# IRVLab/so_dso_place_recognition

Hardware: AMD Instinct MI355X
Metric: queries/sec over 100k-signature DB (SC 20x60, z-score fusion, top-1) (higher is better)
Workload: dtype f16x2 (fp32 carried as f16 hi + lo, fp32 accumulate); binary intensity channel: one f16 product per term, rounded to its exact integer count; 1 GPU; sc_match_100k; db_signatures=100000, descriptor=SC 20x60 x 2 channels, mask_width=0, k=1, db_rows_per_gpu=100000

## Files before the change

so_dso_place_recognition_amd/csrc/kernels.hpp:

```cpp
#pragma once
#include <hip/hip_runtime.h>
#include <stdint.h>

struct pr_ctx;

namespace pr {

constexpr int SC_NF = 31;
constexpr int SC_NSLOT = 16;
constexpr int SC_QIMG = SC_NF * 320;
constexpr int SC_DSTEP = 640;
constexpr int SC_DIMG = 2 * SC_NSLOT * SC_DSTEP;
__host__ __device__ inline int sc_fpos(int f) { return f == 0 ? 0 : (f == 30 ? 1 : f + 1); }
constexpr int SCH_QBLK = 1288;
constexpr int SCH_QIMG = SC_NF * SCH_QBLK;
constexpr int SCH_DTILE = 768;
constexpr int SCH_DFREQ = 4 * SCH_DTILE;
constexpr int SCH_DIMG = SC_NF * SCH_DFREQ;
__host__ __device__ constexpr int sch_qlo_byte(int ring) { return 40 + ((ring + 4) % 20) * 2; }
__host__ __device__ constexpr int sch_a1_byte(int k) { return k == 3 ? 0 : 16 * k; }
__host__ __device__ constexpr int sch_a2_byte(int k) { return k == 0 ? 48 : k == 1 ? 64 : k == 2 ? 32 : 16; }
__host__ __device__ constexpr int sch_b1_byte(int lane) { return lane < 48 ? lane * 16 : SCH_DTILE + (lane - 48) * 16; }
__host__ __device__ constexpr int sch_b2_byte(int lane) { return lane < 32 ? lane * 16 : lane < 48 ? SCH_DTILE + lane * 16 : SCH_DTILE + (lane - 32) * 16; }
constexpr int SCF_QBLK = 640;
constexpr int SCF_QIMG = SC_NF * SCF_QBLK;
constexpr int SCF_DFREQ = 2 * SCH_DTILE;
constexpr int SCF_DIMG = SC_NF * SCF_DFREQ;
constexpr int M2_TILE = 96 * 64;

inline int sc_qgroups8(int m) { return ((m + 31) / 32) * 4; }
inline int sc_qgroups8_f16(int m) { return ((m + 63) / 64) * 8; }
inline int sc_dgroups(int n) { return (n + 15) / 16; }
inline int m2_tiles(int sigs) { return (sigs + 7) / 8; }
inline int m2_qtiles(int sigs) { return ((m2_tiles(sigs) + 11) / 12) * 12; }

constexpr int SC_BSTAT_INTS = 8;
struct ScBin {
  const int* qstat; const int* dstat;
  const float* qinfo; const float* dinfo;
  int* viol;
  int gen;
  float bconst;
  float pair_scale;
  int gate;
  int chsel;
};
#ifdef __HIPCC__
__device__ __forceinline__ bool sc_bin_bound(const ScBin& b, float& bound) {
  const int q0 = b.qstat[0], q1 = b.qstat[1], d0 = b.dstat[0], d1 = b.dstat[1];
  const float eq = __builtin_sqrtf(((__int_as_float(b.qstat[2]) + __int_as_float(b.qstat[3])) + __int_as_float(b.qstat[4])) + __int_as_float(b.qstat[5]));
  const float ed = __builtin_sqrtf(((__int_as_float(b.dstat[2]) + __int_as_float(b.dstat[3])) + __int_as_float(b.dstat[4])) + __int_as_float(b.dstat[5]));
  bound = (eq + ed + eq * ed + b.bconst * (1.f + eq) * (1.f + ed)) * 1.001f;
  return q0 == 0 && d0 == 0 && bound * __builtin_sqrtf((float)q1 * (float)d1) < 0.72f;
}
#endif
void launch_sc_pack(hipStream_t st, const void* sig, int dtype, int rows, int role, float* packed, int groups,
                    const double* twiddle, int* flags, int* bad);
void launch_sc_match(hipStream_t st, const float* qpk, int m, const float* dpk, int n, const float* cst,
                     float* d_p, float* d_i, int nsplit_override);
size_t sc_match_lds_bytes();
void launch_zero_ints(hipStream_t st, int* p, int n);
void launch_fill_ints(hipStream_t st, int* p, int n, int v);
void launch_sc_pack_h(hipStream_t st, const void* sig, int dtype, int rows, int role, void* packed, int groups,
                      const double* twiddle, int* flags, int* bad, int single = 0,
                      float* binfo = nullptr, int* bstat = nullptr);
void launch_sc_pack_h_rows(hipStream_t st, const void* sig, int dtype, int rows, int row0, void* packed, int groups, const double* twiddle,
                           int* flags, int* bad, int single, float* binfo, int* bstat);
void launch_sc_match_h(hipStream_t st, const void* qpk, int m, const void* dpk, int n, const void* cst, float* d_p,
// ... 262 lines not shown
```

so_dso_place_recognition_amd/csrc/sc_match_e.hip:

```cpp
#include <cstdlib>
#include <cstring>

#include "kernels.hpp"
#ifndef E_NO_WAIT1
#define E_WAIT1
#endif
#ifndef E_NO_ACC_OPERANDS
#define E_BACC
#define E_AACC
#define E_SPLIT3
#ifndef E_BD
#define E_BD 5
#endif
#ifndef E_AD
#define E_AD 3
#endif
#ifndef E_PARKR
#define E_PARKR 1
#endif
#endif
#ifndef E_BD
#define E_BD 4
#endif
#ifndef E_BD1
#define E_BD1 8
#endif

namespace pr {
namespace {

typedef _Float16 f16x2 __attribute__((ext_vector_type(2)));
typedef float f32x2 __attribute__((ext_vector_type(2)));
typedef float f32x4 __attribute__((ext_vector_type(4)));
typedef float f32x16 __attribute__((ext_vector_type(16)));
typedef unsigned u32x2 __attribute__((ext_vector_type(2)));
typedef unsigned u32x4 __attribute__((ext_vector_type(4)));
typedef u32x4 u32x4_a8 __attribute__((aligned(8)));

struct AOps { u32x4 h, l; };
struct BOps { u32x4 reh, rel, imh, iml; };
enum { A_H = 0, A_L = 1 };
enum { B_REH = 0, B_REL = 1, B_IMH = 2, B_IML = 3 };

__host__ __device__ constexpr int seqf(int P) { return 16 * (P >> 4) + ((P & 15) >> 1) + 8 * (P & 1); }

typedef const u32x4_a8 __attribute__((address_space(3))) * lds_tile_p;
template <int T>
__device__ __forceinline__ void load_a(AOps& a, unsigned addr) {
  const u32x4 v = *reinterpret_cast<lds_tile_p>(addr);
  if (T == A_H) a.h = v; else a.l = v;
}
template <bool LO, int F, int T, bool SV = false>
__device__ __forceinline__ void load_b(BOps& b, __amdgpu_buffer_rsrc_t rs, int voff) {
  constexpr int soff = LO ? F * SCH_DFREQ : SV ? F * SCH_DFREQ + (T == B_IMH ? 2 : 0) * SCH_DTILE : F * SCF_DFREQ + (T == B_IMH ? 1 : 0) * SCH_DTILE,
                ioff = LO ? ((T == B_IMH || T == B_IML) ? 2 * SCH_DTILE : 0) : 0;
#ifdef E_ABL_ONE_B
  if (!LO && T == B_IMH) { b.imh = b.reh; return; }
#endif
#ifdef E_ABL_B_HOT
  const u32x4 v = __builtin_amdgcn_raw_buffer_load_b128(rs, voff + ioff, 0, 0);
#else
  const u32x4 v = __builtin_amdgcn_raw_buffer_load_b128(rs, voff + ioff, soff, 0);
#endif
  if (T == B_REH) b.reh = v; else if (T == B_REL) b.rel = v; else if (T == B_IMH) b.imh = v; else b.iml = v;
}

#define MF0_(d, a, b, AC, BC) asm volatile("v_mfma_f32_16x16x32_f16 %0, %1, %2, 0" : "=&v"(d) : AC(a), BC(b))
#define MFA_(d, a, b, AC, BC) asm volatile("v_mfma_f32_16x16x32_f16 %0, %1, %2, %0" : "+v"(d) : AC(a), BC(b))
#ifdef E_BACC
#ifdef E_AACC
#define E_AC "a"
#else
#define E_AC "v"
#endif
#define MF0(d, a, b) { if constexpr (LO) MF0_(d, a, b, E_AC, "a"); else MF0_(d, a, b, "v", "v"); }
#define MFA(d, a, b) { if constexpr (LO) MFA_(d, a, b, E_AC, "a"); else MFA_(d, a, b, "v", "v"); }
#else
#define MF0(d, a, b) MF0_(d, a, b, "v", "v")
#define MFA(d, a, b) MFA_(d, a, b, "v", "v")
#endif
#ifndef E_AD
#define E_AD 2
#endif
#ifndef E_PARKR
#define E_PARKR 0
#endif
#ifdef E_BACC
#define E_CC "a"
#else
#define E_CC "v"
#endif
#define M32Z_(d, a, b, AC, BC) asm volatile("v_mfma_f32_32x32x16_f16 %0, %1, %2, 0" : "=&v"(d) : AC(a), BC(b))
#define M32A_(d, a, b, AC, BC) asm volatile("v_mfma_f32_32x32x16_f16 %0, %1, %2, %0" : "+v"(d) : AC(a), BC(b))
#define M32Z(d, a, b, BC) { if constexpr (LO) M32Z_(d, a, b, E_CC, BC); else M32Z_(d, a, b, "v", BC); }
#define M32A(d, a, b, BC) { if constexpr (LO) M32A_(d, a, b, E_CC, BC); else M32A_(d, a, b, "v", BC); }
#define DRAIN() asm volatile("s_nop 9")
#define SB() __builtin_amdgcn_sched_barrier(0)

__device__ __forceinline__ void split2(float x, float y, unsigned& hi, unsigned& lo) {
  const f32x2 v = {x, y};
  hi = __builtin_bit_cast(unsigned, __builtin_convertvector(v, f16x2));
#ifdef E_SPLIT3
// ... 132 lines not shown
    f32x4 (&t)[8] = T[prv];
    if constexpr (G == 0) cmb2(t[0], t[2], t[1], t[3], 2);
    if constexpr (G == 1) { swp2<LO>(t[4], t[6], t[5], t[7], 0); swp2<LO>(t[4], t[6], t[5], t[7], 1); }
    if constexpr (G == 2) cmb2(t[4], t[6], t[5], t[7], 0);
    if constexpr (G == 3) { swp2<LO>(t[4], t[6], t[5], t[7], 2); swp2<LO>(t[4], t[6], t[5], t[7], 3); }
    if constexpr (G == 4) cmb2(t[4], t[6], t[5], t[7], 2);
    if constexpr (G >= 5 && G <= 20) split_piece<LO, PE, ((G - 5) >> 2), ((G - 5) & 3)>(hbs[PH], t);
  }
  if constexpr (QD <= 7) {
    f32x4 (&t)[8] = T[cur];
    if constexpr (G == 21) { swp2<LO>(t[0], t[2], t[1], t[3], 0); swp2<LO>(t[0], t[2], t[1], t[3], 1); }
    if constexpr (G == 22) cmb2(t[0], t[2], t[1], t[3], 0);
    if constexpr (G == 23) { swp2<LO>(t[0], t[2], t[1], t[3], 2); swp2<LO>(t[0], t[2], t[1], t[3], 3); }
  }
}

template <bool LO, int NW, int NQG, bool SV = false>
__global__ __launch_bounds__(64 * NW, NW / 4) void sc_match_e_kernel(const char* __restrict__ qpk,
                                                            const char* __restrict__ dpk,
                                                            const u32x4* __restrict__ cst,
                                                            float* __restrict__ dist_p, float* __restrict__ dist_i,
                                                            int m, int n, int QG8, int DG, int nsplit, ScBin bin,
                                                            int DGS ) {
  extern __shared__ __attribute__((aligned(16))) char lds[];
  static_assert(!SV || !LO, "SV: single-product form");
  float bbound = 0.f;
  if (bin.gate == 0 && bin.chsel == 0 && bin.viol && blockIdx.x == 0 && threadIdx.x == 0) *bin.viol = 0;
  if (bin.gate) {
    const bool pred = sc_bin_bound(bin, bbound);
    if (bin.gate == 1 ? !pred : (pred && *bin.viol != bin.gen)) return;
  }
  [[maybe_unused]] const float bnd25 = bbound * 0x1p25f * bin.pair_scale;
  [[maybe_unused]] int viol = 0;
  const int tid = threadIdx.x, lane = tid & 63;
  const int w = __builtin_amdgcn_readfirstlane(tid >> 6);
  const int xcd = blockIdx.x & 7, idx = blockIdx.x >> 3;
  const int ch = bin.chsel < 0 ? (xcd & 1) : bin.chsel;
  const int range = (bin.chsel < 0 ? (xcd >> 1) + 4 * (idx % nsplit) : xcd + 8 * (idx % nsplit)), qg32 = idx / nsplit;
  const int nrange = (bin.chsel < 0 ? 4 : 8) * nsplit;
  const int g0 = (int)((long long)DG * range / nrange), g1 = (int)((long long)DG * (range + 1) / nrange);

  constexpr int QBLK = LO ? SCH_QBLK : SCF_QBLK, QIMG = LO ? SCH_QIMG : SCF_QIMG, DIMG = (LO || SV) ? SCH_DIMG : SCF_DIMG;
  constexpr int QROW = LO ? 80 : 40;
  static_assert(NW == 4 || !LO, "two waves per SIMD: single-product form only (a split-f16 unit needs all 512 registers)");
  if constexpr (SV) {
    constexpr int WPG = SC_NF * 80;
    unsigned long long* dst = reinterpret_cast<unsigned long long*>(lds);
    for (int i = tid; i < NQG * WPG + 8; i += 64 * NW) {
      const int grp = i / WPG, rem = i - grp * WPG, f = rem / 80, j = rem - f * 80;
      const int gq = qg32 * NQG + grp;
      const int rr = j / 5, c = j - rr * 5;
      unsigned long long v = 0ull;
      if (i < NQG * WPG && gq < QG8)
        v = *reinterpret_cast<const unsigned long long*>(qpk + ((size_t)ch * QG8 + gq) * SCH_QIMG + (size_t)f * SCH_QBLK + rr * 80 + (rr >= 8 ? 8 : 0) + c * 8);
      dst[i] = v;
    }
    float* qi = reinterpret_cast<float*>(lds + NQG * QIMG + 64);
    for (int i = tid; i < 8 * NQG; i += 64 * NW) {
      const int r = qg32 * (8 * NQG) + i;
      qi[2 * i] = r < m ? bin.qinfo[2 * r] * 0x1p-25f : 0.f;
      qi[2 * i + 1] = r < m ? bin.qinfo[2 * r + 1] : 0.f;
    }
  } else {
    const u32x4* src = reinterpret_cast<const u32x4*>(qpk + ((size_t)ch * QG8 + (size_t)qg32 * NQG) * QIMG);
    u32x4* dst = reinterpret_cast<u32x4*>(lds);
    constexpr int NV = NQG * QIMG / 16;
    for (int i = tid; i < NV + 4; i += 64 * NW) dst[i] = (i < NV) ? src[i] : u32x4{0u, 0u, 0u, 0u};
  }
  __syncthreads();

  const int row = lane & 15, kg = lane >> 4;
  const unsigned lds0 = (unsigned)(unsigned long long)(__attribute__((address_space(3))) char*)lds;
  const int wq = w & (NQG - 1), dpar = (NW > NQG) ? (w / NQG) : 0;
  constexpr int GSTEP = NW / NQG;
  const int gcnt = g1 - g0;
  constexpr int BD = LO ? E_BD : E_BD1;
  constexpr int AD = LO ? E_AD : 3;
  const unsigned natr = lds0 + wq * QIMG + row * QROW + ((LO && row >= 8) ? 8 : 0);
  const unsigned nat0 = natr + (LO ? sch_a1_byte(kg) : kg * 16);
  [[maybe_unused]] const unsigned nat1 = natr + sch_a2_byte(kg);
  const int voff = LO ? sch_b1_byte(lane) : ((lane < 48) ? lane * 16 : (int)0x80000000);
  [[maybe_unused]] const int voff2 = sch_b2_byte(lane);
  float* dist = ch ? dist_i : dist_p;
  const char* dbase = dpk + ((size_t)ch * DGS) * DIMG;
  const int qrow0 = qg32 * (8 * NQG) + wq * 8;
  const __amdgpu_buffer_rsrc_t rd = __builtin_amdgcn_make_buffer_rsrc(
      dist + (size_t)qrow0 * n, 0, (qrow0 < m ? (m - qrow0 < 8 ? m - qrow0 : 8) : 0) * n * 4, 0x00020000);
  constexpr int GLINES = SC_NF * 12;
  const int rsd = (LO || NQG == 1) ? 32 : (nsplit >= 32 ? 1 : 32 / nsplit);
  const int pf_slot = (LO || NQG == 1) ? (qg32 & 31) * NW + w : (qg32 % rsd) * NW + w;
  constexpr int PFL = LO ? 6 : 2;
  const int pfl = (LO || NQG == 1) ? PFL : ((NW / NQG) * GLINES + rsd * NW - 1) / (rsd * NW);
  unsigned pf_sink = 0;
  const __amdgpu_buffer_rsrc_t rc = __builtin_amdgcn_make_buffer_rsrc(const_cast<u32x4*>(cst), 0, 8192, 0x00020000);
  if (dpar >= gcnt) return;
  f32x2 qinf[4] = {{0.f, 0.f}, {0.f, 0.f}, {0.f, 0.f}, {0.f, 0.f}};
  if constexpr (SV) {
    const f32x2* qi = reinterpret_cast<const f32x2*>(lds + NQG * QIMG + 64);
#pragma unroll
    for (int r = 0; r < 4; r++) qinf[r] = qi[wq * 8 + r + ((lane & 16) ? 4 : 0)];
  }

  AOps At[AD];
  BOps Bt[BD];
  __amdgpu_buffer_rsrc_t rs =
      __builtin_amdgcn_make_buffer_rsrc(const_cast<char*>(dbase + (size_t)(g0 + dpar) * DIMG), 0, DIMG, 0x00020000);
  constexpr int TPB = LO ? 4 : 2, TPA = LO ? 2 : 1, NREQ = (BD - 1) * TPB + (AD - 1) * TPA;
#define FIRST_REQ(K, RSRC)                                                                                         \
  { if constexpr ((K) < (BD - 1) * TPB) {                                                                          \
      constexpr int _p = (K) / TPB, _t = LO ? (K) % TPB : 2 * ((K) % TPB);       \
      constexpr int _tt = LO ? (_t == 1 ? B_IMH : _t == 2 ? B_REL : _t == 3 ? B_IML : B_REH) : _t;                 \
      load_b<LO, seqf(_p), _tt, SV>(Bt[_p % BD], RSRC, (LO && (_tt == B_REL || _tt == B_IML)) ? voff2 : voff);        \
    } else if constexpr ((K) < NREQ) {                                                                             \
      constexpr int _k = (K) - (BD - 1) * TPB, _p = _k / TPA, _t = _k % TPA;                                       \
      load_a<_t>(At[_p % AD], (_t == A_L ? nat1 : nat0) + seqf(_p) * QBLK);                                        \
    } }
  FIRST_REQ(0, rs) FIRST_REQ(1, rs) FIRST_REQ(2, rs) FIRST_REQ(3, rs) FIRST_REQ(4, rs) FIRST_REQ(5, rs) FIRST_REQ(6, rs) FIRST_REQ(7, rs)
  FIRST_REQ(8, rs) FIRST_REQ(9, rs) FIRST_REQ(10, rs) FIRST_REQ(11, rs) FIRST_REQ(12, rs) FIRST_REQ(13, rs) FIRST_REQ(14, rs) FIRST_REQ(15, rs)
  FIRST_REQ(16, rs) FIRST_REQ(17, rs) FIRST_REQ(18, rs) FIRST_REQ(19, rs) FIRST_REQ(20, rs) FIRST_REQ(21, rs) FIRST_REQ(22, rs) FIRST_REQ(23, rs)
  static_assert(NREQ <= 24, "FIRST_REQ list too short");

  for (int g = g0 + dpar; g < g1; g += GSTEP) {
    const int gn = g + GSTEP;
    const __amdgpu_buffer_rsrc_t rsn =
        __builtin_amdgcn_make_buffer_rsrc(const_cast<char*>(dbase + (size_t)gn * DIMG), 0, DIMG, 0x00020000);
    Half<LO> hbs[2];
    Consts c0, c1;
    f32x4 T[2][8];

#define LDB(Q, TT) { if constexpr ((Q) < 32 && seqf((Q) < 32 ? (Q) : 0) < SC_NF && (LO || (TT == B_REH || TT == B_IMH))) load_b<LO, seqf((Q) < 32 ? (Q) : 0), TT, SV>(Bt[(Q) % BD], rs, (LO && (TT == B_REL || TT == B_IML)) ? voff2 : voff); }
#define LDA(Q, TT) { if constexpr ((Q) < 32 && seqf((Q) < 32 ? (Q) : 0) < SC_NF && (LO || TT == A_H)) load_a<TT>(At[(Q) % AD], (TT == A_L ? nat1 : nat0) + seqf((Q) < 32 ? (Q) : 0) * QBLK); }
#define VS(P, G) valu_slot<LO, ((P) >> 2), (((P) & 3) * 6 + (G))>(T, hbs)
#ifdef E_WAIT1
#ifdef E_WAIT1F
#define TOUCH_OPS_F(P) asm volatile("" : : "v"(At[(P) % AD].h), "v"(Bt[(P) % BD].reh), "v"(Bt[(P) % BD].imh))
#else
#define TOUCH_OPS_F(P)
#endif
#define TOUCH_OPS(P) { if constexpr (LO) asm volatile("" : : "a"(At[(P) % AD].h), "a"(At[(P) % AD].l), "a"(Bt[(P) % BD].reh), "a"(Bt[(P) % BD].imh), "a"(Bt[(P) % BD].rel), "a"(Bt[(P) % BD].iml)); else TOUCH_OPS_F(P); }
#else
#define TOUCH_OPS(P)
#endif
#ifndef E_LDD
#define E_LDD 0
#endif
#ifndef E_VSD
#define E_VSD 0
#endif
#if E_LDD == 0
#define G0_REQ(P) LDA((P) + AD - 1, A_H)
#define G1_REQ(P) LDA((P) + AD - 1, A_L)
#define G2_REQ(P) { LDB((P) + BD - 1, B_REH); LDB((P) + BD - 1, B_IMH); }
#define G3_REQ(P) { LDB((P) + BD - 1, B_REL); LDB((P) + BD - 1, B_IML); }
#else
#define G0_REQ(P) { LDA((P) + AD - 1, A_H); LDB((P) + BD - 1, B_REH); }
#define G1_REQ(P) { LDA((P) + AD - 1, A_L); LDB((P) + BD - 1, B_IMH); }
#define G2_REQ(P) LDB((P) + BD - 1, B_REL)
#define G3_REQ(P) LDB((P) + BD - 1, B_IML)
#endif
#if E_VSD == 0
#define G0_VS(P) VS(P, 0)
#define G1_VS(P) { VS(P, 1); VS(P, 2); }
#define G2_VS(P) VS(P, 3)
#define G3_VS(P) { VS(P, 4); VS(P, 5); }
#elif E_VSD == 1
#define G0_VS(P) { VS(P, 0); VS(P, 1); }
#define G1_VS(P) VS(P, 2)
#define G2_VS(P) { VS(P, 3); VS(P, 4); }
#define G3_VS(P) VS(P, 5)
#elif E_VSD == 2
#define G0_VS(P) VS(P, 0)
#define G1_VS(P) VS(P, 1)
#define G2_VS(P) { VS(P, 2); VS(P, 3); }
#define G3_VS(P) { VS(P, 4); VS(P, 5); }
#else
#define G0_VS(P) { VS(P, 0); VS(P, 1); }
#define G1_VS(P) { VS(P, 2); VS(P, 3); }
#define G2_VS(P) VS(P, 4)
#define G3_VS(P) VS(P, 5)
#endif
#define FREQ(P)                                                                                                  \
  {                                                                                                              \
    f32x4& t1 = T[((P) >> 2) & 1][2 * ((P) & 3)];                                                                \
    f32x4& t2 = T[((P) >> 2) & 1][2 * ((P) & 3) + 1];                                                            \
    if constexpr (seqf(P) < SC_NF && LO) {             \
      SB(); TOUCH_OPS(P); MF0(t1, At[(P) % AD].h, Bt[(P) % BD].reh); SB(); G0_REQ(P); G0_VS(P);                  \
      SB(); MF0(t2, At[(P) % AD].h, Bt[(P) % BD].imh); SB(); G1_REQ(P); G1_VS(P);                                \
      SB(); MFA(t1, At[(P) % AD].l, Bt[(P) % BD].rel); SB(); G2_REQ(P); G2_VS(P);                                \
      SB(); MFA(t2, At[(P) % AD].l, Bt[(P) % BD].iml); SB(); G3_REQ(P); G3_VS(P);                                \
      SB();                                                                                                      \
    } else if constexpr (seqf(P) < SC_NF) {                                                                      \
      SB(); TOUCH_OPS(P); MF0(t1, At[(P) % AD].h, Bt[(P) % BD].reh); SB(); LDA((P) + AD - 1, A_H); VS(P, 0);      \
      SB(); MF0(t2, At[(P) % AD].h, Bt[(P) % BD].imh); SB(); VS(P, 1);                                           \
      SB(); LDB((P) + BD - 1, B_REH); VS(P, 2);                                                                  \
      SB(); LDB((P) + BD - 1, B_IMH); VS(P, 3);                                                                  \
      SB(); VS(P, 4);                                                                                            \
      SB(); VS(P, 5);                                                                                            \
      SB();                                                                                                      \
    } else {                                                                                                     \
      t1 = f32x4{0.f, 0.f, 0.f, 0.f}; t2 = t1;                                        \
      SB(); VS(P, 0); SB(); VS(P, 1); SB(); VS(P, 2); SB(); VS(P, 3); SB(); VS(P, 4); SB(); VS(P, 5); SB();       \
    }                                                                                                            \
  }
    FREQ(0) FREQ(1) FREQ(2) FREQ(3) FREQ(4) FREQ(5) FREQ(6) FREQ(7) FREQ(8) FREQ(9) FREQ(10) FREQ(11) FREQ(12) FREQ(13) FREQ(14) FREQ(15)
    FREQ(16) FREQ(17) FREQ(18) FREQ(19)
    if constexpr (NW == 4) { SB(); park_half<LO>(hbs[0]); SB(); }
    FREQ(20) FREQ(21) FREQ(22) FREQ(23) FREQ(24) FREQ(25) FREQ(26) FREQ(27)
    FREQ(28) FREQ(29)
    load_consts<0, LO>(c0, rc, lane * 16);
    FREQ(30)
    load_consts<1, LO>(c1, rc, lane * 16);
    FREQ(31)
    SB(); DRAIN(); SB();
#define VD(G) valu_slot<LO, 8, G>(T, hbs);
    VD(0) VD(1) VD(2) VD(3) VD(4) VD(5) VD(6) VD(7) VD(8) VD(9) VD(10) VD(11) VD(12) VD(13) VD(14) VD(15) VD(16) VD(17) VD(18) VD(19) VD(20)
    SB();
    {
      asm volatile("" : : "v"(pf_sink));
      const int gp = (g - dpar) + 2 * GSTEP;
      const int pf_bytes = (gp + GSTEP <= DG) ? GSTEP * DIMG : (gp < DG ? (DG - gp) * DIMG : 0);
      const __amdgpu_buffer_rsrc_t rp = __builtin_amdgcn_make_buffer_rsrc(const_cast<char*>(dbase + (size_t)gp * DIMG), 0, pf_bytes, 0x00020000);
      int lp = lane;
      asm volatile("" : "+v"(lp));
      int pf_off = (lp < pfl) ? (pf_slot * pfl + lp) * 128 : (int)0x80000000;
      if constexpr (SV) {
        const int L0 = pf_slot * pfl + lp, gi = L0 / GLINES, L = L0 - gi * GLINES, f = L / 12, r = L - f * 12;
        pf_off = (lp < pfl && gi < GSTEP) ? gi * SCH_DIMG + f * SCH_DFREQ + (r >= 6 ? 2 * SCH_DTILE : 0) + (r >= 6 ? r - 6 : r) * 128 : (int)0x80000000;
      }
      pf_sink = __builtin_amdgcn_raw_buffer_load_b32(rp, pf_off, 0, 0);
    }
    f32x16 tE[2], tO[2];
    float mx = -__builtin_inff();
    int le = lane;
    asm volatile("" : "+v"(le));
    const int st_lane = ((le & 16) ? 4 * n : 0) * 4 + (le & 15) * 4;
    const int st_base = (le < 32 && g * 16 + (le & 15) < n) ? st_lane : (int)0x80000000;
    f32x2 dinf = {0.f, 0.f};
    if constexpr (SV) {
      const int e = g * 16 + (le & 15);
      const float* dp = bin.dinfo + 2 * (size_t)(e < n ? e : 0);
      dinf = f32x2{dp[0], dp[1]};
    }
#define S2I(S, I) s2_one<LO, (NW == 4), ((S) >> 1), ((S) & 1), I>(hbs[0], hbs[1], c0, c1, tE[(S) & 1], tO[(S) & 1])
#define S2G(S, W0, W1, W2, W3, W4, W5, W6, W7, W8, W9, W10, W11)                                   \
  { if constexpr (LO) {                                                                            \
    SB(); S2I(S, 0); SB(); W0;  SB(); S2I(S, 1); SB(); W1;  SB(); S2I(S, 2); SB(); W2;             \
    SB(); S2I(S, 3); SB(); W3;  SB(); S2I(S, 4); SB(); W4;  SB(); S2I(S, 5); SB(); W5;             \
    SB(); S2I(S, 6); SB(); W6;  SB(); S2I(S, 7); SB(); W7;  SB(); S2I(S, 8); SB(); W8;             \
    SB(); S2I(S, 9); SB(); W9;  SB(); S2I(S, 10); SB(); W10; SB(); S2I(S, 11); SB(); W11; SB();    \
  } else {                                                                                         \
    SB(); S2I(S, 0); SB(); W0; W1; W2; SB(); S2I(S, 1); SB(); S2I(S, 2); SB(); W3; W4; W5;         \
    W6; W7; W8; SB(); S2I(S, 3); SB(); W9; W10; W11; SB(); } }
#define RP(S, i) { if constexpr (!LO && (i) == 0) asm volatile("" : "+v"(tE[(S) & 1]), "+v"(tO[(S) & 1])); mx = red_piece(mx, tE[(S) & 1], tO[(S) & 1], i); }
#define ST(S) { if constexpr (SV) ep_store_round(mx, qinf[(S) >> 1], dinf, bnd25, viol, rd, st_base + ((S) >> 1) * 4 * n + g * 64);   \
                else ep_store(mx, rd, st_base + ((S) >> 1) * 4 * n + g * 64);                                                  \
                mx = -__builtin_inff(); }
#define NX(K) FIRST_REQ(K, rsn)
#define NONE ((void)0)
    S2G(0, NONE, NONE, NONE, NONE, NONE, NONE, NONE, NONE, NONE, NONE, NONE, NONE)
    S2G(1, NX(16), NX(17), NX(18), RP(0, 0), RP(0, 1), RP(0, 2), RP(0, 3), RP(0, 4), RP(0, 5), RP(0, 6), RP(0, 7), NX(19))
    S2G(2, NX(0), NX(1), NX(20), RP(1, 0), RP(1, 1), RP(1, 2), RP(1, 3), RP(1, 4), RP(1, 5), RP(1, 6), RP(1, 7), ST(1))
    S2G(3, NX(2), NX(3), NX(4), RP(2, 0), RP(2, 1), RP(2, 2), RP(2, 3), RP(2, 4), RP(2, 5), RP(2, 6), RP(2, 7), NX(22))
    S2G(4, NX(5), NX(6), NX(21), RP(3, 0), RP(3, 1), RP(3, 2), RP(3, 3), RP(3, 4), RP(3, 5), RP(3, 6), RP(3, 7), ST(3))
    S2G(5, NX(7), NX(8), NX(9), RP(4, 0), RP(4, 1), RP(4, 2), RP(4, 3), RP(4, 4), RP(4, 5), RP(4, 6), RP(4, 7), NX(23))
// ... 123 lines not shown
```

so_dso_place_recognition_amd/csrc/sc_match_h.hip:

```cpp
#include "kernels.hpp"

namespace pr {
namespace {

typedef _Float16 f16x2 __attribute__((ext_vector_type(2)));
typedef _Float16 f16x8 __attribute__((ext_vector_type(8)));
typedef float f32x2 __attribute__((ext_vector_type(2)));
typedef float f32x4 __attribute__((ext_vector_type(4)));
typedef float f32x16 __attribute__((ext_vector_type(16)));
typedef unsigned u32x2 __attribute__((ext_vector_type(2)));
typedef unsigned u32x4 __attribute__((ext_vector_type(4)));
typedef u32x4 u32x4_a8 __attribute__((aligned(8)));

struct AOps { u32x4 h, l, rh, rl; };
struct BOps { u32x4 reh, rel, imh, iml; };

enum { A_H = 0, A_L = 1, A_RH = 2, A_RL = 3 };
enum { B_REH = 0, B_REL = 1, B_IMH = 2, B_IML = 3 };
typedef const u32x4_a8 __attribute__((address_space(3))) * lds_tile_p;
template <int P, int T>
__device__ __forceinline__ void load_a(AOps& a, unsigned nat, unsigned rot, unsigned dl) {
  unsigned addr = ((T & 2) ? rot : nat) + (P & 1) * SCH_QBLK;
  if (T & 1) addr += dl;
  const u32x4 v = *reinterpret_cast<lds_tile_p>(addr);
// ... 87 lines not shown
template <int R>
__device__ __forceinline__ void ep_elem(float& mx, const f32x16 (&accE)[4][2], const f32x16 (&accO)[4][2], int e) {
  const float vf = accE[R][0][e] + __builtin_fabsf(accO[R][0][e]);
  const float vm = accE[R][1][e] + __builtin_fabsf(accO[R][1][e]);
  mx = fmaxf(fmaxf(mx, vf), vm);
}
template <int R>
__device__ __forceinline__ void ep_store(float mx, __amdgpu_buffer_rsrc_t rd, int st_off) {
  const u32x2 sw = __builtin_amdgcn_permlane32_swap(__float_as_uint(mx), __float_as_uint(mx), false, false);
  mx = fmaxf(__uint_as_float(sw[0]), __uint_as_float(sw[1]));
  __builtin_amdgcn_raw_buffer_store_b32(__float_as_uint(__builtin_fmaf(mx, -0x1p-26f, 0.5f)), rd, st_off, 0, 0);
}

#define FM2(F, M, t1, t2, r0)                                                        \
  {                                                                                  \
    const f32x2 _a = {t1[r0], t1[r0 + 1]}, _b = {t2[r0], t2[r0 + 1]};                \
    const f32x2 _f = __builtin_elementwise_fma(_b, sg2, _a), _m = __builtin_elementwise_fma(_b, -sg2, _a); \
    F[r0] = _f[0]; F[r0 + 1] = _f[1]; M[r0] = _m[0]; M[r0 + 1] = _m[1];             \
  }

template <bool ONEQ>
__global__ __launch_bounds__(256, 1) void sc_match_h_kernel(const char* __restrict__ qpk,
                                                            const char* __restrict__ dpk,
                                                            const u32x4* __restrict__ cst,
                                                            float* __restrict__ dist_p, float* __restrict__ dist_i,
                                                            int m, int n, int QG8, int DG, int nsplit, ScBin bin) {
  extern __shared__ __attribute__((aligned(16))) char lds[];
  if (bin.gate == 0 && bin.chsel == 0 && bin.viol && blockIdx.x == 0 && threadIdx.x == 0) *bin.viol = 0;
  if (bin.gate == 2) {
    float bound;
    if (sc_bin_bound(bin, bound) && *bin.viol != bin.gen) return;
  }
  const int tid = threadIdx.x, lane = tid & 63;
  const int w = __builtin_amdgcn_readfirstlane(tid >> 6);
  const int xcd = blockIdx.x & 7, idx = blockIdx.x >> 3;
  const int ch = bin.chsel < 0 ? (xcd & 1) : bin.chsel;
  const int range = (bin.chsel < 0 ? (xcd >> 1) + 4 * (idx % nsplit) : xcd + 8 * (idx % nsplit)), qg32 = idx / nsplit;
  const int nrange = (bin.chsel < 0 ? 4 : 8) * nsplit;
  const int g0 = (int)((long long)DG * range / nrange), g1 = (int)((long long)DG * (range + 1) / nrange);

  {
    const u32x4* src = reinterpret_cast<const u32x4*>(qpk + ((size_t)ch * QG8 + (size_t)qg32 * 4) * SCH_QIMG);
    u32x4* dst = reinterpret_cast<u32x4*>(lds);
    constexpr int NV = 4 * SCH_QIMG / 16;
    for (int i = tid; i < NV + 4; i += 256) dst[i] = (i < NV) ? src[i] : u32x4{0u, 0u, 0u, 0u};
  }
  __syncthreads();
  if (g0 >= g1) return;

  const int row = lane & 15, kg = lane >> 4;
  const unsigned lds0 = (unsigned)(unsigned long long)(__attribute__((address_space(3))) char*)lds;
  constexpr int GS = ONEQ ? 4 : 1;
  const int wq = ONEQ ? 0 : w;
  const unsigned nat0 = lds0 + wq * SCH_QIMG + row * 80 + (row >= 8 ? 8 : 0) + sch_a1_byte(kg);
  const unsigned rot0 = lds0 + wq * SCH_QIMG + (row ^ 8) * 80 + (row >= 8 ? 0 : 8) + sch_a1_byte(kg);
  const unsigned dl = sch_a2_byte(kg) - sch_a1_byte(kg);
  const int voff = sch_b1_byte(lane), voff2 = sch_b2_byte(lane);
  const float sg = (lane < 32) ? 1.0f : -1.0f;
  const f32x2 sg2 = {sg, sg};
  float* dist = ch ? dist_i : dist_p;
  const char* dbase = dpk + ((size_t)ch * DG) * SCH_DIMG;
  const f32x16 zero = {0.f, 0.f, 0.f, 0.f, 0.f, 0.f, 0.f, 0.f, 0.f, 0.f, 0.f, 0.f, 0.f, 0.f, 0.f, 0.f};
  const int qrow0 = qg32 * 32 + wq * 8;
  const __amdgpu_buffer_rsrc_t rd = __builtin_amdgcn_make_buffer_rsrc(
      dist + (size_t)qrow0 * n, 0, (qrow0 < m ? (m - qrow0 < 8 ? m - qrow0 : 8) : 0) * n * 4, 0x00020000);
  const int pf_slot = (qg32 & 31) * 4 + w;
  unsigned pf_sink = 0;
  const __amdgpu_buffer_rsrc_t rc = __builtin_amdgcn_make_buffer_rsrc(const_cast<u32x4*>(cst), 0, 8192, 0x00020000);

  AOps At[4];
  BOps Bt[4];
  __amdgpu_buffer_rsrc_t rs =
      __builtin_amdgcn_make_buffer_rsrc(const_cast<char*>(dbase + (size_t)(g0 + (ONEQ ? w : 0)) * SCH_DIMG), 0, SCH_DIMG, 0x00020000);
  load_b<0, B_REH>(Bt[0], rs, voff, voff2); load_b<0, B_IMH>(Bt[0], rs, voff, voff2); load_b<0, B_REL>(Bt[0], rs, voff, voff2); load_b<0, B_IML>(Bt[0], rs, voff, voff2);
  load_a<0, A_H>(At[0], nat0, rot0, dl); load_a<0, A_RH>(At[0], nat0, rot0, dl); load_a<0, A_L>(At[0], nat0, rot0, dl); load_a<0, A_RL>(At[0], nat0, rot0, dl);
  load_b<1, B_REH>(Bt[1], rs, voff, voff2); load_b<1, B_IMH>(Bt[1], rs, voff, voff2); load_b<1, B_REL>(Bt[1], rs, voff, voff2);
  load_a<1, A_H>(At[1], nat0, rot0, dl); load_a<1, A_RH>(At[1], nat0, rot0, dl);
#ifdef PR_SCH_TIMING
  unsigned long long tacc[8] = {0, 0, 0, 0, 0, 0, 0, 0}, tprev;
  asm volatile("s_memtime %0\n\ts_waitcnt lgkmcnt(0)" : "=s"(tprev));
#endif
  unsigned nbase = nat0, rbase = rot0;
  for (int g = g0 + (ONEQ ? w : 0); g < g1; g += GS) {
    const __amdgpu_buffer_rsrc_t rsn =
        __builtin_amdgcn_make_buffer_rsrc(const_cast<char*>(dbase + (size_t)(g + GS) * SCH_DIMG), 0, SCH_DIMG, 0x00020000);
    f32x16 accE[4][2], accO[4][2];
    Half hb;
    Consts c;
    f32x4 Fa, Ma, Fb, Mb, t1a, t2a, t1b, t2b;
    unsigned ncur, rcur, nnxt = nbase, rnxt = rbase;
    TICK(7)
#define LDB(Q, T) { if ((Q) < SC_NF) load_b<((Q) < SC_NF ? (Q) : 0), T>(Bt[(Q) & 3], rs, voff, voff2); }
#define LDA(P, Q, T) { if ((Q) < SC_NF) { if (((Q) >> 1) == ((P) >> 1)) load_a<((Q) < SC_NF ? (Q) : 0), T>(At[(Q) & 3], ncur, rcur, dl); \
                                        else load_a<((Q) < SC_NF ? (Q) : 0), T>(At[(Q) & 3], nnxt, rnxt, dl); } }
#define FREQ(P, t1, t2, W0, W1, W2, W3, W4, W5)                                                   \
  {                                                                                               \
    SB(); MF0(t1, At[(P) & 3].h, Bt[(P) & 3].reh);  SB(); LDB((P) + 1, B_IML); LDA(P, (P) + 1, A_L); W0;   \
    SB(); MF0(t2, At[(P) & 3].rh, Bt[(P) & 3].imh); SB(); LDB((P) + 2, B_REH); W1;                \
    SB(); MFA(t1, At[(P) & 3].l, Bt[(P) & 3].rel);  SB(); LDB((P) + 2, B_IMH); LDA(P, (P) + 1, A_RL); W2; LDA(P, (P) + 2, A_H); W3;  \
    SB(); MFA(t2, At[(P) & 3].rl, Bt[(P) & 3].iml); SB(); LDB((P) + 2, B_REL); W4; LDA(P, (P) + 2, A_RH); W5;              \
    SB();                                                                                         \
  }
#define PKF(J, R) pack_F<J, R>(hb, Fa, Fb)
#define PKM(J, R) pack_M<J, R>(hb, Ma, Mb)
#define PK(J, R) { PKF(J, R); PKM(J, R); }
#define NONE ((void)0)
#define ADV() { ncur = nnxt; rcur = rnxt; nnxt = ncur + 2 * SCH_QBLK; rnxt = rcur + 2 * SCH_QBLK; asm("" : "+v"(nnxt)); asm("" : "+v"(rnxt)); }
#define FMA_ALL(F, M, t1, t2) { FM2(F, M, t1, t2, 0); FM2(F, M, t1, t2, 2); }
// ... 130 lines not shown
```

so_dso_place_recognition_amd/csrc/sc_pack.hip:

```cpp
#include <cstdlib>
#include <cstring>

#include "kernels.hpp"

namespace pr {
namespace {

constexpr int SC_PACK_FEW = 8;

template <typename T>
__global__ __launch_bounds__(256) void sc_pack_kernel(const T* __restrict__ sig, int rows, int role,
                                                       float* __restrict__ packed, int groups,
                                                       const double* __restrict__ tw, int* __restrict__ flags,
                                                       int* __restrict__ bad) {
  __shared__ double x[1200];
  __shared__ double red[256];
  __shared__ double tws[120];
  const int tid = threadIdx.x;
  const int row = blockIdx.x >> 1, ch = blockIdx.x & 1;
  const T* src = sig + (size_t)row * 2400 + ch * 1200;
  double part = 0.0;
  for (int i = tid; i < 1200; i += 256) {
    double v = (double)src[i];
    x[i] = v;
// ... 44 lines not shown
__global__ __launch_bounds__(320) void sc_pack_h_kernel(const T* __restrict__ sig, int rows, int role,
                                                         unsigned short* __restrict__ packed, int groups,
                                                         const double* __restrict__ tw, int* __restrict__ flags,
                                                         int* __restrict__ bad) {
  __shared__ double x[1200];
  __shared__ double red[320];
  __shared__ double tws[120];
  const int tid = threadIdx.x;
  const int row = blockIdx.x >> 1, ch = blockIdx.x & 1;
  const T* src = sig + (size_t)row * 2400 + ch * 1200;
  double part = 0.0;
  for (int i = tid; i < 1200; i += 320) {
    double v = (double)src[i];
    x[i] = v;
    part += v * v;
  }
  if (tid < 120) tws[tid] = tw[tid];
  red[tid] = part;
  __syncthreads();
  if (tid < 64) red[tid] += red[tid + 256];
  __syncthreads();
  for (int s = 128; s > 0; s >>= 1) {
    if (tid < s) red[tid] += red[tid + s];
    __syncthreads();
  }
  const double nr = sqrt(red[0]);
  const bool isbad = !(nr > 0.0) || !(nr < __builtin_inf());
  if (tid == 0) { bad[2 * row + ch] = isbad ? (1 << ch) : 0; if (isbad) atomicOr(flags, 1); }
  for (int i = tid; i < 1200; i += 320) x[i] = isbad ? 0.0 : x[i] / nr;
  __syncthreads();
  const double scale = 0.12909944487358055 * (role == 0 ? 256.0 : 128.0);
  {
    const int o = tid;
    const int f = o / 20, ring = o - f * 20;
    double ce = 0.0, co = 0.0, se = 0.0, so = 0.0;
    int t = 0;
#pragma unroll 3
    for (int s2 = 0; s2 < 60; s2 += 2) {
      const double x0 = x[s2 * 20 + ring];
      ce += x0 * tws[t];
      se += x0 * tws[60 + t];
      t += f; if (t >= 60) t -= 60;
      const double x1 = x[(s2 + 1) * 20 + ring];
      co += x1 * tws[t];
      so += x1 * tws[60 + t];
      t += f; if (t >= 60) t -= 60;
    }
    auto put = [&](double val, int ff, int im) {
      const _Float16 hi = (_Float16)val;
      const _Float16 lo = (_Float16)(val - (double)hi);
      size_t bh, bl;
      if (role == 0) {
        const int g = row >> 3, rr = (im << 3) | (row & 7);
        const size_t base = ((size_t)ch * groups + g) * SCH_QIMG + (size_t)ff * SCH_QBLK + rr * 80 + (rr >= 8 ? 8 : 0);
        bh = base + ring * 2;
        bl = base + sch_qlo_byte(ring);
      } else {
        const int g = row >> 4, j = row & 15;
        const size_t base = ((size_t)ch * groups + g) * SCH_DIMG + (size_t)ff * SCH_DFREQ + (size_t)im * 2 * SCH_DTILE +
                            (((ring >> 3) << 4) | j) * 16 + (ring & 7) * 2;
        bh = base;
        bl = base + SCH_DTILE;
        if (ring >= 16) packed[(bl + 8) >> 1] = __builtin_bit_cast(unsigned short, hi);
      }
      packed[bh >> 1] = __builtin_bit_cast(unsigned short, hi);
      packed[bl >> 1] = __builtin_bit_cast(unsigned short, lo);
    };
    put((ce + co) * scale, f, 0);
    put(-(se + so) * scale, f, 1);
    if (f != 15) {
      put((ce - co) * scale, 30 - f, 0);
      put((se - so) * scale, 30 - f, 1);
    }
  }
}

template <typename T, int ROLE, bool LO>
__global__ __launch_bounds__(320) void sc_pack_h_col_kernel(const T* __restrict__ sig, int rows,
                                                             unsigned short* __restrict__ packed, int groups,
                                                             const double* __restrict__ tw, int* __restrict__ flags,
                                                             int* __restrict__ bad, float* __restrict__ binfo, int* __restrict__ bstat) {
  constexpr int SL = ROLE == 0 ? (LO ? SCH_QBLK : SCF_QBLK) : (LO ? SCH_DFREQ : SCF_DFREQ);
  constexpr int NG = ROLE == 0 ? 2 : 1;
  constexpr int IMGB = ROLE == 0 ? (LO ? SCH_QIMG : SCF_QIMG) : (LO ? SCH_DIMG : SCF_DIMG);
  constexpr int QROW = LO ? 80 : 40;
  __shared__ __attribute__((aligned(16))) char img[NG * 8 * SL];
  __shared__ double part[16 * 20];
  __shared__ int bnz[LO ? 320 : 1];
  __shared__ float epart[LO ? 320 : 1];
  const int tid = threadIdx.x, lrow = tid / 20, ring = tid - 20 * lrow;
  const int xcd = blockIdx.x & 7, idx = blockIdx.x >> 3;
  const int fb = idx & 3, ch = (idx >> 2) & 1, blk = (idx >> 3) * 8 + xcd;
  if (blk * 16 >= rows) return;
  const int row = blk * 16 + lrow;
  const bool valid = row < rows;
  for (int i = tid; i < NG * 8 * SL / 8; i += 320) reinterpret_cast<unsigned long long*>(img)[i] = 0ull;
  const T* src = sig + (size_t)(valid ? row : 0) * 2400 + ch * 1200 + ring;
  double ce[4] = {0, 0, 0, 0}, co[4] = {0, 0, 0, 0}, se[4] = {0, 0, 0, 0}, so[4] = {0, 0, 0, 0};
  double nsq = 0.0;
  const bool do_eps = LO && binfo != nullptr && ch == 1, do_bin = do_eps && fb == 0;
  int nz = 0;
  double vmn = __builtin_inf(), vmx = -__builtin_inf();
  float e2 = 0.f;
  const double* twc = tw + 120 + (size_t)fb * 60 * 8;
#ifndef SCP_AHEAD
#define SCP_AHEAD 2
#endif
// ... 36 lines not shown
  if (LO && do_bin) bnz[tid] = (nz == 0 || (vmn == vmx && vmn > 0.0)) ? nz : -1;
  __syncthreads();
  double n2 = 0.0;
#pragma unroll
  for (int r = 0; r < 20; r++) n2 += part[lrow * 20 + r];
  const double nr = sqrt(n2);
  const bool isbad = !(nr > 0.0) || !(nr < __builtin_inf());
  if (valid && ring == 0 && fb == 0) { bad[2 * row + ch] = isbad ? (1 << ch) : 0; if (isbad) atomicOr(flags, 1); }
  const int srow = blk * 16 + tid;
  bool sbad = true;
  if (LO && do_eps && tid < 16) {
    double n2t = 0.0;
#pragma unroll
    for (int r = 0; r < 20; r++) n2t += part[tid * 20 + r];
    const double nrt = sqrt(n2t);
    sbad = srow >= rows || !(nrt > 0.0) || !(nrt < __builtin_inf());
  }
  if (LO && do_bin) {
    __syncthreads();
    part[tid] = vmx;
    __syncthreads();
    if (tid < 16) {
      int ones = 0;
      bool binary = true;
      double a = -__builtin_inf();
      for (int r = 0; r < 20; r++) {
        const int c = bnz[tid * 20 + r];
        const double v = part[tid * 20 + r];
        if (c < 0) binary = false;
        if (c > 0) { ones += c; if (a == -__builtin_inf()) a = v; else if (v != a) binary = false; }
      }
      binary = binary && ones > 0;
      float s1 = 1.f, rs = 1.f;
      if (!sbad && binary) { s1 = (float)sqrt((double)ones); rs = (float)(1.0 / sqrt((double)ones)); }
      if (srow < rows) { binfo[2 * srow] = s1; binfo[2 * srow + 1] = rs; }
      int mo = (!sbad && binary) ? ones : 0, nb = (!sbad && !binary) ? 1 : 0;
#pragma unroll
      for (int o = 8; o > 0; o >>= 1) { mo = max(mo, __shfl_xor(mo, o)); nb |= __shfl_xor(nb, o); }
      if (tid == 0) { bstat[SC_BSTAT_INTS + 6 * blk] = nb; bstat[SC_BSTAT_INTS + 6 * blk + 1] = mo; }
    }
  }
  const double sc = isbad ? 0.0 : 0.12909944487358055 * (ROLE == 0 ? 256.0 : 128.0) / nr;
  auto put = [&](double val, int slice, int im) {
    if (isbad) val = 0.0;
    float vf = (float)val;
    asm volatile("" : "+v"(vf));
    const _Float16 hi = (_Float16)vf;
    float rf = (float)(val - (double)hi);
    asm volatile("" : "+v"(rf));
    const _Float16 lo = (_Float16)rf;
    int bh, bl;
    if (ROLE == 0) {
      const int rr = (im << 3) | (lrow & 7);
      bh = ((lrow >> 3) * 8 + slice) * SL + rr * QROW + ((LO && rr >= 8) ? 8 : 0) + ring * 2;
      bl = bh - ring * 2 + sch_qlo_byte(ring);
    } else {
      bh = slice * SL + im * (LO ? 2 : 1) * SCH_DTILE + (((ring >> 3) << 4) | lrow) * 16 + (ring & 7) * 2;
      bl = bh + SCH_DTILE;
      if (LO && ring >= 16) *reinterpret_cast<_Float16*>(img + bl + 8) = hi;
    }
    *reinterpret_cast<_Float16*>(img + bh) = hi;
    if (LO) *reinterpret_cast<_Float16*>(img + bl) = lo;
    if (LO) {
      const bool edge = (fb == 0 && (slice & 3) == 0);
      e2 = __builtin_fmaf(edge ? rf : 2.f * rf, rf, e2);
    }
  };
  if (valid) {
#pragma unroll
    for (int j = 0; j < 4; j++) {
      put((ce[j] + co[j]) * sc, j, 0);
      put(-(se[j] + so[j]) * sc, j, 1);
      if (4 * fb + j != 15) {
        put((ce[j] - co[j]) * sc, 4 + j, 0);
        put((se[j] - so[j]) * sc, 4 + j, 1);
      }
    }
  }
  if (LO && do_eps) epart[tid] = e2;
  __syncthreads();
  if (LO && do_eps && tid < 16) {
    float e = 0.f;
    for (int r = 0; r < 20; r++) e += epart[tid * 20 + r];
    if (sbad) e = 0.f;
#pragma unroll
    for (int o = 8; o > 0; o >>= 1) e = fmaxf(e, __shfl_xor(e, o));
    const int eb = __float_as_int(e * (ROLE == 0 ? 0x1p-16f : 0x1p-14f) * (1.f + 0x1p-10f));
    if (tid == 0) bstat[SC_BSTAT_INTS + 6 * blk + 2 + fb] = eb;
  }
  constexpr int W = SL / 8;
  for (int i = tid; i < NG * 8 * W; i += 320) {
    const int sl = i / W, wd = i - sl * W, gg = sl >> 3, k = sl & 7;
    const int f = k < 4 ? 4 * fb + k : 30 - 4 * fb - (k - 4);
    if (k >= 4 && f == 15) continue;
    const int g = NG * blk + gg;
    if (g >= groups) continue;
    reinterpret_cast<unsigned long long*>(reinterpret_cast<char*>(packed) + ((size_t)ch * groups + g) * IMGB + (size_t)f * SL)[wd] =
        reinterpret_cast<const unsigned long long*>(img)[i];
  }
}

__device__ __forceinline__ double wave_sum(double v) {
#pragma unroll
  for (int o = 32; o > 0; o >>= 1) v += __shfl_xor(v, o);
  return v;
}
template <typename T, int ROLE, bool LO>
// ... 24 lines not shown
    if ((tid & 63) == 0) { wred[tid >> 6][0] = bz; wred[tid >> 6][1] = bmn_; wred[tid >> 6][2] = bmx_; }
  }
  if (tid < 120) tws[tid] = tw[tid];
  __syncthreads();
  double ce = 0.0, co = 0.0, se = 0.0, so = 0.0, nsq = 0.0;
  int t = 0;
#pragma unroll 1
  for (int s2 = 0; s2 < 60; s2 += 2) {
    const double x0 = x[s2 * 20 + ring], x1 = x[(s2 + 1) * 20 + ring];
    nsq += x0 * x0;
    nsq += x1 * x1;
    ce += x0 * tws[t];
    se += x0 * tws[60 + t];
    t += f; if (t >= 60) t -= 60;
    co += x1 * tws[t];
    so += x1 * tws[60 + t];
    t += f; if (t >= 60) t -= 60;
  }
  if (f == 0) part[ring] = nsq;
  __syncthreads();
  double n2 = 0.0;
#pragma unroll
  for (int r = 0; r < 20; r++) n2 += part[r];
  const double nr = sqrt(n2);
  const bool isbad = !(nr > 0.0) || !(nr < __builtin_inf());
  if (tid == 0) { bad[2 * row + ch] = isbad ? (1 << ch) : 0; if (isbad) atomicOr(flags, 1); }
  if (do_bin && tid == 0) {
    double ones = 0.0, mn = __builtin_inf(), mx = -__builtin_inf();
    for (int w5 = 0; w5 < 5; w5++) { ones += wred[w5][0]; mn = fmin(mn, wred[w5][1]); mx = fmax(mx, wred[w5][2]); }
    const bool binary = ones > 0.0 && mn == mx && mn > 0.0;
    float s = 1.f, rs = 1.f;
    if (!isbad && binary) { s = (float)sqrt(ones); rs = (float)(1.0 / sqrt(ones)); atomicMax(bstat + 1, (int)ones); }
    if (!isbad && !binary) atomicOr(bstat, 1);
    binfo[2 * row] = s; binfo[2 * row + 1] = rs;
  }
  const double sc = isbad ? 0.0 : 0.12909944487358055 * (ROLE == 0 ? 256.0 : 128.0) / nr;
  char* out = reinterpret_cast<char*>(packed);
  double e2 = 0.0;
  auto put = [&](double val, int ff, int im) {
    if (isbad) val = 0.0;
    float vf = (float)val;
    asm volatile("" : "+v"(vf));
    const _Float16 hi = (_Float16)vf;
    float rf = (float)(val - (double)hi);
    asm volatile("" : "+v"(rf));
    const _Float16 lo = (_Float16)rf;
    if (do_bin) {
      const double r = (val - (double)hi) * (ROLE == 0 ? 0x1p-8 : 0x1p-7);
      e2 += ((ff == 0 || ff == 30) ? 1.0 : 2.0) * r * r;
    }
    size_t bh;
    if (ROLE == 0) {
      const int g = row >> 3, rr = (im << 3) | (row & 7);
      bh = ((size_t)ch * groups + g) * IMGB + (size_t)ff * SL + rr * QROW + ((LO && rr >= 8) ? 8 : 0) + ring * 2;
      *reinterpret_cast<_Float16*>(out + bh) = hi;
      if (LO) *reinterpret_cast<_Float16*>(out + bh - ring * 2 + sch_qlo_byte(ring)) = lo;
    } else {
      const int g = row >> 4, j = row & 15;
      bh = ((size_t)ch * groups + g) * IMGB + (size_t)ff * SL + (size_t)im * (LO ? 2 : 1) * SCH_DTILE + (((ring >> 3) << 4) | j) * 16 + (ring & 7) * 2;
      *reinterpret_cast<_Float16*>(out + bh) = hi;
      if (LO) *reinterpret_cast<_Float16*>(out + bh + SCH_DTILE) = lo;
      if (LO && ring >= 16) *reinterpret_cast<_Float16*>(out + bh + SCH_DTILE + 8) = hi;
    }
  };
  put((ce + co) * sc, f, 0);
  put(-(se + so) * sc, f, 1);
  if (f != 15) {
    put((ce - co) * sc, 30 - f, 0);
    put((se - so) * sc, 30 - f, 1);
  }
  if (do_bin) {
    e2 = wave_sum(e2);
    __syncthreads();
    if ((tid & 63) == 0) wred[tid >> 6][0] = e2;
    __syncthreads();
    if (tid == 0 && !isbad) {
      double e = 0.0;
      for (int w5 = 0; w5 < 5; w5++) e += wred[w5][0];
      atomicMax(bstat + 2, __float_as_int((float)(e * (1.0 + 0x1p-20))));
    }
  }
}

__global__ __launch_bounds__(256) void sc_bstat_finalize_kernel(int* __restrict__ bstat, int nblk) {
  __shared__ int red[6][256];
  int v[6] = {0, 0, 0, 0, 0, 0};
  for (int b = threadIdx.x; b < nblk; b += 256) {
    const int* w = bstat + SC_BSTAT_INTS + 6 * b;
    v[0] |= w[0];
#pragma unroll
    for (int i = 1; i < 6; i++) v[i] = max(v[i], w[i]);
  }
#pragma unroll
  for (int i = 0; i < 6; i++) red[i][threadIdx.x] = v[i];
  __syncthreads();
  for (int s2 = 128; s2 > 0; s2 >>= 1) {
    if ((int)threadIdx.x < s2) {
      red[0][threadIdx.x] |= red[0][threadIdx.x + s2];
#pragma unroll
      for (int i = 1; i < 6; i++) red[i][threadIdx.x] = max(red[i][threadIdx.x], red[i][threadIdx.x + s2]);
    }
    __syncthreads();
  }
  if (threadIdx.x < 6) bstat[threadIdx.x] = red[threadIdx.x][0];
}

template <typename T, int ROLE, bool LO = true>
// ... 82 lines not shown
```

Baseline: 138,100 queries/s.

## Align split-f16 query rows to 16 bytes, permute rows, hoist constants into AGPRs

The split-f16 query tile layout changes from 80-byte rows with an 8-byte offset for the upper half (1288-byte blocks) to 16-byte-aligned 80-byte rows placed by a fixed row permutation. The permutation is presumably chosen to avoid LDS bank conflicts, and the alignment lets A-operand loads use fully aligned ds_read_b128. The per-lane constants are loaded once before the DB loop and pinned in accumulator registers, where they used to be reloaded every iteration. The B prefetch depth also goes from 5 to 6. This costs extra AGPR pressure, and every packer and consumer has to agree on the new row mapping.

```diff
diff --git a/so_dso_place_recognition_amd/csrc/kernels.hpp b/so_dso_place_recognition_amd/csrc/kernels.hpp
--- a/so_dso_place_recognition_amd/csrc/kernels.hpp
+++ b/so_dso_place_recognition_amd/csrc/kernels.hpp
@@ -12,8 +12,12 @@
 constexpr int SC_DSTEP = 640;
 constexpr int SC_DIMG = 2 * SC_NSLOT * SC_DSTEP;
 __host__ __device__ inline int sc_fpos(int f) { return f == 0 ? 0 : (f == 30 ? 1 : f + 1); }
-constexpr int SCH_QBLK = 1288;
+constexpr int SCH_QROW = 80;
+constexpr int SCH_QBLK = 16 * SCH_QROW;
 constexpr int SCH_QIMG = SC_NF * SCH_QBLK;
+__host__ __device__ constexpr int sch_qrow_pos(int row) { return (int)((0xedbafc9865327410ull >> (4 * row)) & 15); }
+__host__ __device__ constexpr int sch_qrow_byte(int row) { return SCH_QROW * sch_qrow_pos(row); }
+static_assert(SCH_QROW % 16 == 0 && SCH_QBLK % 16 == 0 && SCH_QIMG % 16 == 0, "ds_read_b128 needs 16-byte aligned query tiles");
 constexpr int SCH_DTILE = 768;
 constexpr int SCH_DFREQ = 4 * SCH_DTILE;
 constexpr int SCH_DIMG = SC_NF * SCH_DFREQ;
diff --git a/so_dso_place_recognition_amd/csrc/sc_match_e.hip b/so_dso_place_recognition_amd/csrc/sc_match_e.hip
--- a/so_dso_place_recognition_amd/csrc/sc_match_e.hip
+++ b/so_dso_place_recognition_amd/csrc/sc_match_e.hip
@@ -10,7 +10,7 @@
 #define E_AACC
 #define E_SPLIT3
 #ifndef E_BD
-#define E_BD 5
+#define E_BD 6
 #endif
 #ifndef E_AD
 #define E_AD 3
@@ -44,10 +44,12 @@
 
 __host__ __device__ constexpr int seqf(int P) { return 16 * (P >> 4) + ((P & 15) >> 1) + 8 * (P & 1); }
 
-typedef const u32x4_a8 __attribute__((address_space(3))) * lds_tile_p;
-template <int T>
+typedef const u32x4 __attribute__((address_space(3))) * lds_tile_p;
+typedef const u32x4_a8 __attribute__((address_space(3))) * lds_tile_a8_p;
+template <int T, bool LO>
 __device__ __forceinline__ void load_a(AOps& a, unsigned addr) {
-  const u32x4 v = *reinterpret_cast<lds_tile_p>(addr);
+  u32x4 v;
+  if constexpr (LO) v = *reinterpret_cast<lds_tile_p>(addr); else v = *reinterpret_cast<lds_tile_a8_p>(addr);
   if (T == A_H) a.h = v; else a.l = v;
 }
 template <bool LO, int F, int T, bool SV = false>
@@ -286,7 +288,7 @@
       const int rr = j / 5, c = j - rr * 5;
       unsigned long long v = 0ull;
       if (i < NQG * WPG && gq < QG8)
-        v = *reinterpret_cast<const unsigned long long*>(qpk + ((size_t)ch * QG8 + gq) * SCH_QIMG + (size_t)f * SCH_QBLK + rr * 80 + (rr >= 8 ? 8 : 0) + c * 8);
+        v = *reinterpret_cast<const unsigned long long*>(qpk + ((size_t)ch * QG8 + gq) * SCH_QIMG + (size_t)f * SCH_QBLK + sch_qrow_byte(rr) + c * 8);
       dst[i] = v;
     }
     float* qi = reinterpret_cast<float*>(lds + NQG * QIMG + 64);
@@ -310,7 +312,8 @@
   const int gcnt = g1 - g0;
   constexpr int BD = LO ? E_BD : E_BD1;
   constexpr int AD = LO ? E_AD : 3;
-  const unsigned natr = lds0 + wq * QIMG + row * QROW + ((LO && row >= 8) ? 8 : 0);
+  static_assert(!LO || (QIMG % 16 == 0 && QBLK % 16 == 0 && QROW % 16 == 0), "split-f16 query tiles are read with ds_read_b128");
+  const unsigned natr = lds0 + wq * QIMG + (LO ? sch_qrow_byte(row) : row * QROW);
   const unsigned nat0 = natr + (LO ? sch_a1_byte(kg) : kg * 16);
   [[maybe_unused]] const unsigned nat1 = natr + sch_a2_byte(kg);
   const int voff = LO ? sch_b1_byte(lane) : ((lane < 48) ? lane * 16 : (int)0x80000000);
@@ -335,6 +338,8 @@
     for (int r = 0; r < 4; r++) qinf[r] = qi[wq * 8 + r + ((lane & 16) ? 4 : 0)];
   }
 
+  Consts c0, c1;
+  if constexpr (LO) { load_consts<0, LO>(c0, rc, lane * 16); load_consts<1, LO>(c1, rc, lane * 16); }
   AOps At[AD];
   BOps Bt[BD];
   __amdgpu_buffer_rsrc_t rs =
@@ -347,7 +352,7 @@
       load_b<LO, seqf(_p), _tt, SV>(Bt[_p % BD], RSRC, (LO && (_tt == B_REL || _tt == B_IML)) ? voff2 : voff);        \
     } else if constexpr ((K) < NREQ) {                                                                             \
       constexpr int _k = (K) - (BD - 1) * TPB, _p = _k / TPA, _t = _k % TPA;                                       \
-      load_a<_t>(At[_p % AD], (_t == A_L ? nat1 : nat0) + seqf(_p) * QBLK);                                        \
+      load_a<_t, LO>(At[_p % AD], (_t == A_L ? nat1 : nat0) + seqf(_p) * QBLK);                                    \
     } }
   FIRST_REQ(0, rs) FIRST_REQ(1, rs) FIRST_REQ(2, rs) FIRST_REQ(3, rs) FIRST_REQ(4, rs) FIRST_REQ(5, rs) FIRST_REQ(6, rs) FIRST_REQ(7, rs)
   FIRST_REQ(8, rs) FIRST_REQ(9, rs) FIRST_REQ(10, rs) FIRST_REQ(11, rs) FIRST_REQ(12, rs) FIRST_REQ(13, rs) FIRST_REQ(14, rs) FIRST_REQ(15, rs)
@@ -359,11 +364,12 @@
     const __amdgpu_buffer_rsrc_t rsn =
         __builtin_amdgcn_make_buffer_rsrc(const_cast<char*>(dbase + (size_t)gn * DIMG), 0, DIMG, 0x00020000);
     Half<LO> hbs[2];
-    Consts c0, c1;
     f32x4 T[2][8];
+    if constexpr (LO)
+      asm volatile("" : "+a"(c0.ch), "+a"(c0.cl), "+a"(c0.sh), "+a"(c0.sl), "+a"(c1.ch), "+a"(c1.cl), "+a"(c1.sh), "+a"(c1.sl));
 
 #define LDB(Q, TT) { if constexpr ((Q) < 32 && seqf((Q) < 32 ? (Q) : 0) < SC_NF && (LO || (TT == B_REH || TT == B_IMH))) load_b<LO, seqf((Q) < 32 ? (Q) : 0), TT, SV>(Bt[(Q) % BD], rs, (LO && (TT == B_REL || TT == B_IML)) ? voff2 : voff); }
-#define LDA(Q, TT) { if constexpr ((Q) < 32 && seqf((Q) < 32 ? (Q) : 0) < SC_NF && (LO || TT == A_H)) load_a<TT>(At[(Q) % AD], (TT == A_L ? nat1 : nat0) + seqf((Q) < 32 ? (Q) : 0) * QBLK); }
+#define LDA(Q, TT) { if constexpr ((Q) < 32 && seqf((Q) < 32 ? (Q) : 0) < SC_NF && (LO || TT == A_H)) load_a<TT, LO>(At[(Q) % AD], (TT == A_L ? nat1 : nat0) + seqf((Q) < 32 ? (Q) : 0) * QBLK); }
 #define VS(P, G) valu_slot<LO, ((P) >> 2), (((P) & 3) * 6 + (G))>(T, hbs)
 #ifdef E_WAIT1
 #ifdef E_WAIT1F
@@ -441,9 +447,9 @@
     if constexpr (NW == 4) { SB(); park_half<LO>(hbs[0]); SB(); }
     FREQ(20) FREQ(21) FREQ(22) FREQ(23) FREQ(24) FREQ(25) FREQ(26) FREQ(27)
     FREQ(28) FREQ(29)
-    load_consts<0, LO>(c0, rc, lane * 16);
+    if constexpr (!LO) load_consts<0, LO>(c0, rc, lane * 16);
     FREQ(30)
-    load_consts<1, LO>(c1, rc, lane * 16);
+    if constexpr (!LO) load_consts<1, LO>(c1, rc, lane * 16);
     FREQ(31)
     SB(); DRAIN(); SB();
 #define VD(G) valu_slot<LO, 8, G>(T, hbs);
diff --git a/so_dso_place_recognition_amd/csrc/sc_match_h.hip b/so_dso_place_recognition_amd/csrc/sc_match_h.hip
--- a/so_dso_place_recognition_amd/csrc/sc_match_h.hip
+++ b/so_dso_place_recognition_amd/csrc/sc_match_h.hip
@@ -163,8 +163,8 @@
   const unsigned lds0 = (unsigned)(unsigned long long)(__attribute__((address_space(3))) char*)lds;
   constexpr int GS = ONEQ ? 4 : 1;
   const int wq = ONEQ ? 0 : w;
-  const unsigned nat0 = lds0 + wq * SCH_QIMG + row * 80 + (row >= 8 ? 8 : 0) + sch_a1_byte(kg);
-  const unsigned rot0 = lds0 + wq * SCH_QIMG + (row ^ 8) * 80 + (row >= 8 ? 0 : 8) + sch_a1_byte(kg);
+  const unsigned nat0 = lds0 + wq * SCH_QIMG + sch_qrow_byte(row) + sch_a1_byte(kg);
+  const unsigned rot0 = lds0 + wq * SCH_QIMG + sch_qrow_byte(row ^ 8) + sch_a1_byte(kg);
   const unsigned dl = sch_a2_byte(kg) - sch_a1_byte(kg);
   const int voff = sch_b1_byte(lane), voff2 = sch_b2_byte(lane);
   const float sg = (lane < 32) ? 1.0f : -1.0f;
diff --git a/so_dso_place_recognition_amd/csrc/sc_pack.hip b/so_dso_place_recognition_amd/csrc/sc_pack.hip
--- a/so_dso_place_recognition_amd/csrc/sc_pack.hip
+++ b/so_dso_place_recognition_amd/csrc/sc_pack.hip
@@ -120,7 +120,7 @@
       size_t bh, bl;
       if (role == 0) {
         const int g = row >> 3, rr = (im << 3) | (row & 7);
-        const size_t base = ((size_t)ch * groups + g) * SCH_QIMG + (size_t)ff * SCH_QBLK + rr * 80 + (rr >= 8 ? 8 : 0);
+        const size_t base = ((size_t)ch * groups + g) * SCH_QIMG + (size_t)ff * SCH_QBLK + sch_qrow_byte(rr);
         bh = base + ring * 2;
         bl = base + sch_qlo_byte(ring);
       } else {
@@ -263,7 +263,7 @@
     int bh, bl;
     if (ROLE == 0) {
       const int rr = (im << 3) | (lrow & 7);
-      bh = ((lrow >> 3) * 8 + slice) * SL + rr * QROW + ((LO && rr >= 8) ? 8 : 0) + ring * 2;
+      bh = ((lrow >> 3) * 8 + slice) * SL + (LO ? sch_qrow_byte(rr) : rr * QROW) + ring * 2;
       bl = bh - ring * 2 + sch_qlo_byte(ring);
     } else {
       bh = slice * SL + im * (LO ? 2 : 1) * SCH_DTILE + (((ring >> 3) << 4) | lrow) * 16 + (ring & 7) * 2;
@@ -394,7 +394,7 @@
     size_t bh;
     if (ROLE == 0) {
       const int g = row >> 3, rr = (im << 3) | (row & 7);
-      bh = ((size_t)ch * groups + g) * IMGB + (size_t)ff * SL + rr * QROW + ((LO && rr >= 8) ? 8 : 0) + ring * 2;
+      bh = ((size_t)ch * groups + g) * IMGB + (size_t)ff * SL + (LO ? sch_qrow_byte(rr) : rr * QROW) + ring * 2;
       *reinterpret_cast<_Float16*>(out + bh) = hi;
       if (LO) *reinterpret_cast<_Float16*>(out + bh - ring * 2 + sch_qlo_byte(ring)) = lo;
     } else {
```

After: 140,400 queries/s, median of 6. 1.02x the previous value.
